# mosesyhc/LCGP

Hardware: AMD Instinct MI355X
Metric: NLL+grad evals/sec (higher is better)
Workload: dtype f64; 1 GPU; configs[2]: n=4096 d=6 p=64 q=8 submethod=full, one NLL+gradient evaluation per step; n=4096, d=6, p=64, q=8, parallelism=latent components k -> rank k mod 1, q_local_rank0=8

## Files before the change

lcgp_amd/csrc/lcgp_hip.hip:

```cpp
#include <hip/hip_runtime.h>
#include <stdint.h>
#include <stdio.h>
#include <string.h>
#include <math.h>
#include <type_traits>
#include <vector>

#include "../../include/lcgp_hip.h"
#include "fill_sched.h"
#include "sobol_subset.h"

#define LCGP_VERSION 610

namespace {

constexpr int TS = 64;
constexpr int KT = 16;
constexpr int DMAX = 32;
constexpr int DWIDE = 126;

typedef double d4 __attribute__((ext_vector_type(4)));
typedef float f4 __attribute__((ext_vector_type(4)));

thread_local char g_err[256] = "";
// ... 376 lines not shown
        out[(size_t)gi * ldo + gj] = (T)v;
    }
}

constexpr double MARG_SERIES_BELOW = 0.5;
constexpr int MARG_SERIES_TERMS = 20;

template <int KERN>
__device__ __forceinline__ void marg_series(double b, double& F, double& G) {
    double t = 1.0, sf = 0.0, sg = 0.0;
    for (int m = 0; m < MARG_SERIES_TERMS; ++m) {
        const double f = KERN == 0 ? 1.0 - m : (m - 1.0) * (m - 3.0) / 3.0;
        sf += t * f / (m + 1.0);
        sg += t * f / (m + 2.0);
        t *= -b / (m + 1.0);
    }
    F = b * sf;
    G = b * b * sg;
}

template <int KERN>
__device__ __forceinline__ double marg_F(double b) {
    if constexpr (KERN == 1) {
        return 1.2533141373155003 * erf(b * 0.70710678118654752);
    } else {
        if (b < MARG_SERIES_BELOW) { double F, G; marg_series<KERN>(b, F, G); return F; }
        const double e = exp(-b), em = -expm1(-b);
        if constexpr (KERN == 0) return 2.0 * em - b * e;
        else return (8.0 / 3.0) * em - b * (5.0 + b) / 3.0 * e;
    }
}

template <int KERN>
__device__ __forceinline__ double marg_G(double b) {
    if constexpr (KERN == 1) {
        return -expm1(-0.5 * b * b);
    } else {
        if (b < MARG_SERIES_BELOW) { double F, G; marg_series<KERN>(b, F, G); return G; }
        const double e = exp(-b), em = -expm1(-b);
        if constexpr (KERN == 0) return 3.0 * em - b * (3.0 + b) * e;
        else return 5.0 * em - b * (5.0 + b * (2.0 + b / 3.0)) * e;
    }
}

template <int KERN>
__device__ __forceinline__ double marg_Fc(double b) {
    if constexpr (KERN == 0) return (2.0 + b) * exp(-b);
    else if constexpr (KERN == 1) return 1.2533141373155003 * erfc(b * 0.70710678118654752);
    else return (8.0 + b * (5.0 + b)) / 3.0 * exp(-b);
}

template <int KERN>
__device__ __forceinline__ double marg_I1(double xv, double lo, double hi, double ell) {
    const double w = hi - lo;
    const double a1 = xv - lo, a2 = hi - xv;
    const double b1 = fabs(a1) / ell, b2 = fabs(a2) / ell;
    double r;
    if (a1 >= 0.0 && a2 >= 0.0) {
        r = marg_F<KERN>(b1) + marg_F<KERN>(b2);
    } else {
        const double bn = fmin(b1, b2), bf = fmax(b1, b2);
        r = bn > 1.0 ? marg_Fc<KERN>(bn) - marg_Fc<KERN>(bf) : marg_F<KERN>(bf) - marg_F<KERN>(bn);
    }
    return ell / w * r;
}

template <typename T, int KERN>
__global__ __launch_bounds__(256) void marg_table_kernel(const T* __restrict__ x, int n, int npad, int d,
                                                         const double* __restrict__ theta, int tw,
                                                         const double* __restrict__ box ,
                                                         double* __restrict__ tab, double* __restrict__ i2) {
    const int j = blockIdx.x * 256 + threadIdx.x, l = blockIdx.y, k = blockIdx.z;
    const double ell = theta[(size_t)k * tw + l];
    const double lo = box[l], hi = box[d + l], w = hi - lo;
    if (j == 0) {
        const double a = w / ell;
        i2[(size_t)k * d + l] = 2.0 * (marg_F<KERN>(a) / a - marg_G<KERN>(a) / (a * a));
    }
    if (j >= npad) return;
    double v = 1.0;
    if (j < n) {
        v = marg_I1<KERN>((double)x[(size_t)j * d + l], lo, hi, ell);
    }
    tab[((size_t)k * d + l) * npad + j] = v;
}

__device__ __forceinline__ double fast_rcp(double a) {
    double x = __builtin_amdgcn_rcp(a);
    x = fma(fma(-a, x, 1.0), x, x);
    x = fma(fma(-a, x, 1.0), x, x);
    return x;
}

template <int C>
__device__ __forceinline__ double row_bcast(double x) {
    double o;
    asm("s_nop 1\n\tv_mov_b64_dpp %0, %1 row_newbcast:%2 row_mask:0xf bank_mask:0xf" : "=v"(o) : "v"(x), "n"(C));
    return o;
}

template <int C>
__device__ __forceinline__ void fmac_row_bcast(double& acc, double u, double v) {
    asm("v_fmac_f64_dpp %0, %1, %2 row_newbcast:%3 row_mask:0xf bank_mask:0xf" : "+v"(acc) : "v"(u), "v"(v), "n"(C));
}

template <int S, int C>
struct PivotCols {
    static __device__ __forceinline__ void run(double (&rD)[16], double (&rL)[16], double vD, double vL) {
        if constexpr (C < 16) {
            fmac_row_bcast<C>(rD[C], rD[S], vD);
            fmac_row_bcast<C>(rL[C], rD[S], vL);
            PivotCols<S, C + 1>::run(rD, rL, vD, vL);
        }
    }
};

template <int S>
struct PivotSteps {
    static __device__ __forceinline__ void run(double (&rD)[16], double (&rL)[16], double& dmine, int i) {
        if constexpr (S < 16) {
            const double dp = row_bcast<S>(rD[S]);
            dmine = i == S ? rD[S] : dmine;
            const double rdp = fast_rcp(dp);
            const double vD = -rD[S] * rdp, vL = -rL[S] * rdp;
            PivotCols<S, S + 1>::run(rD, rL, vD, vL);
            PivotSteps<S + 1>::run(rD, rL, dmine, i);
        }
    }
};

template <int S>
struct ScaleCols {
    static __device__ __forceinline__ void run(double (&rD)[16], double (&rL)[16], double rsl) {
        if constexpr (S < 16) {
            const double f = row_bcast<S>(rsl);
            rD[S] *= f;
            rL[S] *= f;
            ScaleCols<S + 1>::run(rD, rL, rsl);
        }
    }
};

__device__ __forceinline__ double fast_rsqrt(double a) {
    double y = __builtin_amdgcn_rsq(a);
    double e = fma(-(a * y), y, 1.0);
    y = fma(0.5 * y, e, y);
    e = fma(-(a * y), y, 1.0);
    y = fma(0.5 * y, e, y);
    return y;
}

constexpr int LEAF_LDT = TS + 1;
constexpr int LEAF_SCR = TS * 17;
constexpr int LEAF_LDS_BYTES = (2 * TS * LEAF_LDT + LEAF_SCR + 2 * TS) * 8 + 16;

__device__ __forceinline__ void leaf_inverse_diag(double (*lt)[LEAF_LDT], double (*w)[LEAF_LDT], const double* dinv, int a,
                                                  int lane) {
    if (lane < 16) {
        const int b0 = a * 16, cl = lane;
        double wc[16];
#pragma unroll
        for (int i = 0; i < 16; ++i) {
            double sacc = i == cl ? -1.0 : 0.0;
#pragma unroll
            for (int m = 0; m < i; ++m) sacc = fma(lt[b0 + m][b0 + i], wc[m], sacc);
            wc[i] = -sacc * dinv[b0 + i];
        }
#pragma unroll
        for (int i = 0; i < 16; ++i) w[b0 + i][b0 + cl] = wc[i];
    }
}

__device__ __forceinline__ d4 leaf_inverse_t(double (*lt)[LEAF_LDT], double (*w)[LEAF_LDT], int a, int b, int lane) {
    const int li = lane & 15, lq = lane >> 4;
    d4 tacc = {0.0, 0.0, 0.0, 0.0};
    for (int mb = b; mb < a; ++mb) {
#pragma unroll
        for (int st = 0; st < 4; ++st)
            tacc = __builtin_amdgcn_mfma_f64_16x16x4f64(lt[mb * 16 + 4 * st + lq][a * 16 + li], w[mb * 16 + 4 * st + lq][b * 16 + li],
                                                        tacc, 0, 0, 0);
    }
    return tacc;
}

__device__ __forceinline__ void leaf_inverse_w(double (*w)[LEAF_LDT], const d4& tacc, int a, int b, int lane) {
    const int li = lane & 15, lq = lane >> 4;
    d4 wacc = {0.0, 0.0, 0.0, 0.0};
#pragma unroll
    for (int st = 0; st < 4; ++st)
        wacc = __builtin_amdgcn_mfma_f64_16x16x4f64(w[a * 16 + li][a * 16 + 4 * st + lq], tacc[st], wacc, 0, 0, 0);
#pragma unroll
    for (int e = 0; e < 4; ++e) w[a * 16 + lq + 4 * e][b * 16 + li] = -wacc[e];
}

template <typename T>
__device__ __forceinline__ void leaf_store_l_panel(T* __restrict__ Mb, int npad, double (*lt)[LEAF_LDT], int pb, int lane) {
    const int col = pb * 16 + (lane & 15);
#pragma unroll
    for (int m = 0; m < 16; ++m) {
        const int i = (lane >> 4) + 4 * m;
        Mb[(size_t)i * npad + col] = (T)lt[col][i];
    }
}

template <typename T>
__device__ __forceinline__ void leaf_store_w_rows(T* __restrict__ Wb, int npad, double (*w)[LEAF_LDT], int a, int lane) {
#pragma unroll
    for (int m = 0; m < 16; ++m) {
        const int i = a * 16 + m;
        Wb[(size_t)i * npad + lane] = (T)(lane <= i ? w[i][lane] : 0.0);
    }
}

template <typename T, bool FROM_LDS>
__device__ __forceinline__ void leaf_factor_invert(T* __restrict__ Mb, T* __restrict__ Wb, int npad, double (*lt)[LEAF_LDT],
                                                   double (*w)[LEAF_LDT], double* scratch, double* dinv, double* pivs,
                                                   int* bad, int jb) {
    const int tid = body_tid(), lane = tid & 63, wv = __builtin_amdgcn_readfirstlane(tid >> 6);
    const int li = lane & 15, lq = lane >> 4;
    d4 acc[4];
#pragma unroll
    for (int rb = 0; rb < 4; ++rb)
#pragma unroll
        for (int e = 0; e < 4; ++e)
            acc[rb][e] = rb < wv ? 0.0 : FROM_LDS ? w[rb * 16 + lq + 4 * e][wv * 16 + li]
                                                  : (double)Mb[(size_t)(rb * 16 + lq + 4 * e) * npad + wv * 16 + li];
    double (*S)[17] = (double (*)[17])scratch;
    int first_bad = 0;
#pragma unroll 1
    for (int kb = 0; kb < 4; ++kb) {
        if (wv == kb) {
#pragma unroll
            for (int rb = 0; rb < 4; ++rb)
#pragma unroll
                for (int e = 0; e < 4; ++e)
                    if (rb >= kb) S[rb * 16 + lq + 4 * e][li] = acc[rb][e];
            const int nlow = 3 - kb;
            const int base = kb * 16;
            double rD[16], rL[16];
            const int lrow = lq < nlow ? base + 16 * (1 + lq) + li : base + li;
#pragma unroll
            for (int c = 0; c < 16; ++c) {
                rD[c] = S[base + li][c];
                const double below = S[lrow][c];
                rL[c] = lq < nlow ? below : 0.0;
            }
            double dmine = 1.0;
            PivotSteps<0>::run(rD, rL, dmine, li);
            const double rsl = fast_rsqrt(dmine);
            ScaleCols<0>::run(rD, rL, rsl);
            if (lq == 0) { dinv[base + li] = rsl; pivs[base + li] = dmine; }
            const unsigned long long bm = __ballot(!(dmine > 0.0)) & 0xffffull;
            if (bm) first_bad = jb * TS + base + __ffsll((long long)bm);
            const int row = lq < nlow ? base + 16 * (1 + lq) + li : lq == nlow ? base + li : 16 * (lq - nlow - 1) + li;
#pragma unroll
            for (int m = 0; m < 16; ++m)
                lt[base + m][row] = lq < nlow ? rL[m] : (lq == nlow && li >= m) ? rD[m] : 0.0;
            if (lane == 0) bad[kb] = first_bad;
        } else if (wv == kb - 1) {
            const int a = kb - 1;
            leaf_inverse_diag(lt, w, dinv, a, lane);
            for (int b = 0; b < a; ++b) {
                const d4 tacc = leaf_inverse_t(lt, w, a, b, lane);
                leaf_inverse_w(w, tacc, a, b, lane);
            }
        } else if (kb == 0) {
            if ((jb & 1) == 0)
                for (int i = wv - 1; i < TS; i += 3) Wb[(size_t)i * npad + TS + lane] = (T)0;
        } else if (wv == ((kb + 1) & 3)) {
            leaf_store_l_panel<T>(Mb, npad, lt, kb - 1, lane);
        } else if (kb >= 2 && wv == ((kb + 2) & 3)) {
            leaf_store_w_rows<T>(Wb, npad, w, kb - 2, lane);
        }
        __syncthreads();
        if (wv > kb) {
#pragma unroll
            for (int st = 0; st < 4; ++st) {
                const double bv = lt[kb * 16 + 4 * st + lq][wv * 16 + li];
#pragma unroll
                for (int rb = 1; rb < 4; ++rb)
                    if (rb >= wv)
                        acc[rb] = __builtin_amdgcn_mfma_f64_16x16x4f64(-lt[kb * 16 + 4 * st + lq][rb * 16 + li], bv, acc[rb],
                                                                       0, 0, 0);
            }
        }
    }
    d4 tacc = {0.0, 0.0, 0.0, 0.0};
    if (wv == 3) leaf_inverse_diag(lt, w, dinv, 3, lane);
    else tacc = leaf_inverse_t(lt, w, 3, wv, lane);
    __syncthreads();
    if (wv < 3) leaf_inverse_w(w, tacc, 3, wv, lane);
    else leaf_store_l_panel<T>(Mb, npad, lt, 3, lane);
    __syncthreads();
    if (wv == 1) leaf_store_w_rows<T>(Wb, npad, w, 2, lane);
    else if (wv == 2) leaf_store_w_rows<T>(Wb, npad, w, 3, lane);
}

template <typename T, bool FROM_LDS = false>
__device__ __forceinline__ void leaf_body(unsigned char* lds, int k, T* __restrict__ M, T* __restrict__ W, size_t mat,
                                          int npad, int jb, double* __restrict__ logdet, int* __restrict__ info) {
    double (*lt)[LEAF_LDT] = (double (*)[LEAF_LDT])lds;
    double (*w)[LEAF_LDT] = (double (*)[LEAF_LDT])((double*)lds + TS * LEAF_LDT);
    double* scratch = (double*)lds + 2 * TS * LEAF_LDT;
    double* dinv = scratch + LEAF_SCR;
    double* pivs = dinv + TS;
    int* bad = (int*)(pivs + TS);
    const int tid = body_tid();
    T* Mb = M + (size_t)k * mat + (size_t)jb * TS * npad + (size_t)jb * TS;
    T* Wb = W + (size_t)k * mat + (size_t)jb * TS * npad + (size_t)jb * TS;
    double ld_prev = 0.0;
    int info_prev = 0;
    if (tid == 0) { ld_prev = logdet[k]; info_prev = info[k]; }
    leaf_factor_invert<T, FROM_LDS>(Mb, Wb, npad, lt, w, scratch, dinv, pivs, bad, jb);
    if (tid < TS) {
        double lg = 0.5 * log(pivs[tid]);
        for (int off = 32; off > 0; off >>= 1) lg += __shfl_xor(lg, off);
        if (tid == 0) {
            logdet[k] = ld_prev + lg;
            const int fb = bad[0] ? bad[0] : bad[1] ? bad[1] : bad[2] ? bad[2] : bad[3];
            if (fb && info_prev == 0) info[k] = fb;
        }
    }
}

template <typename T>
__global__ __launch_bounds__(256, 2) void leaf_kernel(T* __restrict__ M, T* __restrict__ W, size_t mat, int npad, int jb,
                                                   double* __restrict__ logdet, int* __restrict__ info) {
    __shared__ __align__(16) unsigned char lds[LEAF_LDS_BYTES];
    leaf_body<T>(lds, blockIdx.x, M, W, mat, npad, jb, logdet, info);
}

enum GemmOp { OP_SYRK = 1, OP_TRTRI_T = 2, OP_TRTRI_W = 3, OP_LAUUM = 4, OP_PRED_U = 5, OP_PRED_COV = 6, OP_PRED_V = 7, OP_VR = 8,
              OP_VG_P = 9, OP_VG_G = 10, OP_HESS_G = 11, OP_COND_CROSS = 12, OP_COND_U = 13 };
enum Lay { MK = 0, KM = 1 };

struct GemmArgs {
    const void* A; const void* B; void* C;
    size_t sA, sB, sC;
    int ldA, ldB, ldC;
    int nb;
    int p0, p1, p2, p3;
    int q;
    int t0;
    int skipq;
    const void* bvec = nullptr;
    double* part = nullptr;
    unsigned long long* clk = nullptr;
    const double* theta = nullptr;
    const void* xa = nullptr;
    const void* xb = nullptr;
    const double* wref = nullptr;
    const double* gvc = nullptr;
    int ldg = 0, d = 0, kern = 0, tw = 0, nrep = 1, ldp = 0;
};

template <typename T>
__device__ __forceinline__ constexpr int lds_swz(int k) { return (k & 12) * (int)(8 / sizeof(T)); }
static_assert(KT == 16, "lds_swz assumes 16 k rows per stage");
template <typename T>
__device__ __forceinline__ int swz_col(int g16, int l15, int kk) {
    return (g16 ^ (lds_swz<T>(4 * kk) & ~15)) + (l15 ^ (lds_swz<T>(4 * kk) & 15));
}

template <typename T, int L, int TM, int NT>
__device__ __forceinline__ void load_stage(const T* __restrict__ P, int ld, int ks, T (&reg)[TM * KT / NT], int tid) {
    constexpr int EPT = TM * KT / NT;
    if (L == MK) {
        constexpr int TPR = KT / EPT;
        const int m = tid / TPR, kk = (tid % TPR) * EPT;
        const T* src = P + (size_t)m * ld + ks + kk;
#pragma unroll
        for (int e = 0; e < EPT; ++e) reg[e] = src[e];
    } else {
        constexpr int TPK = TM / EPT;
        constexpr int PE = 16 / (int)sizeof(T), NP = EPT / PE;
        const int kq = tid / TPK, j = tid % TPK;
        const T* src = P + (size_t)(ks + kq) * ld + j * PE;
#pragma unroll
        for (int pc = 0; pc < NP; ++pc)
#pragma unroll
            for (int e = 0; e < PE; ++e) reg[pc * PE + e] = src[pc * (TM / NP) + e];
    }
}

template <typename T, int L, int TM, int NT>
__device__ __forceinline__ void store_stage(T* __restrict__ S, const T (&reg)[TM * KT / NT], int tid) {
    constexpr int EPT = TM * KT / NT;
    constexpr int LD = TM + 16;
    if (L == MK) {
        constexpr int TPR = KT / EPT;
        const int m = tid / TPR, kk = (tid % TPR) * EPT;
#pragma unroll
        for (int e = 0; e < EPT; ++e) S[(kk + e) * LD + (m ^ lds_swz<T>(kk + e))] = reg[e];
    } else {
        constexpr int TPK = TM / EPT;
        constexpr int PE = 16 / (int)sizeof(T), NP = EPT / PE;
        const int kq = tid / TPK, j = tid % TPK;
#pragma unroll
        for (int pc = 0; pc < NP; ++pc)
#pragma unroll
            for (int e = 0; e < PE; ++e) S[kq * LD + ((j * PE + pc * (TM / NP)) ^ lds_swz<T>(kq)) + e] = reg[pc * PE + e];
    }
}

template <typename T> struct Piece;
template <> struct Piece<double> { typedef double v __attribute__((ext_vector_type(2))); };
template <> struct Piece<float> { typedef float v __attribute__((ext_vector_type(4))); };

template <int IMM, typename P>
__device__ __forceinline__ void gload_piece(P& dst, unsigned voff, const void* sbase) {
    asm volatile("global_load_dwordx4 %0, %1, %2 offset:%3" : "=v"(dst) : "v"(voff), "s"(sbase), "n"(IMM) : "memory");
}

template <int N, typename P>
__device__ __forceinline__ void vm_wait_set(P (&a)[1], P (&b)[1]) {
    asm volatile("s_waitcnt vmcnt(%2)" : "+v"(a[0]), "+v"(b[0]) : "n"(N) : "memory");
}
template <int N, typename P>
__device__ __forceinline__ void vm_wait_set(P (&a)[4], P (&b)[4]) {
    asm volatile("s_waitcnt vmcnt(%8)" : "+v"(a[0]), "+v"(a[1]), "+v"(a[2]), "+v"(a[3]), "+v"(b[0]), "+v"(b[1]), "+v"(b[2]), "+v"(b[3])
                 : "n"(N) : "memory");
}
template <int N, typename P>
__device__ __forceinline__ void vm_wait_set(P (&a)[2], P (&b)[2]) {
    asm volatile("s_waitcnt vmcnt(%4)" : "+v"(a[0]), "+v"(a[1]), "+v"(b[0]), "+v"(b[1]) : "n"(N) : "memory");
}

template <typename T, int L, int TM, int NT>
__device__ __forceinline__ unsigned stage_lane_offset(int ld, int tid) {
    constexpr int EPT = TM * KT / NT;
    constexpr int PE = 16 / (int)sizeof(T);
    if (L == MK) {
        constexpr int TPR = KT / EPT;
        const int m = tid / TPR, kk = (tid % TPR) * EPT;
        return (unsigned)((m * ld + kk) * (int)sizeof(T));
    } else {
        constexpr int TPK = TM / EPT;
        const int kq = tid / TPK, j = tid % TPK;
        return (unsigned)((kq * ld + j * PE) * (int)sizeof(T));
    }
}

template <typename T, int L, int TM, int NT>
__device__ __forceinline__ void load_stage_u(const T* __restrict__ P , int ld, int ks, T (&reg)[TM * KT / NT],
                                             unsigned voff) {
    constexpr int EPT = TM * KT / NT;
    const T* src = (const T*)((const char*)(L == MK ? P + ks : P + (size_t)ks * ld) + voff);
    if (L == MK) {
#pragma unroll
        for (int e = 0; e < EPT; ++e) reg[e] = src[e];
    } else {
        constexpr int PE = 16 / (int)sizeof(T), NP = EPT / PE;
#pragma unroll
        for (int pc = 0; pc < NP; ++pc)
#pragma unroll
            for (int e = 0; e < PE; ++e) reg[pc * PE + e] = src[pc * (TM / NP) + e];
    }
}

template <typename T, int L, int TM, int NT, int PC = 0>
__device__ __forceinline__ void load_stage_p(const T* __restrict__ P , int ld, int ks,
                                             typename Piece<T>::v (&reg)[TM * KT / NT * (int)sizeof(T) / 16], unsigned voff) {
    constexpr int EPT = TM * KT / NT;
    constexpr int PE = 16 / (int)sizeof(T), NP = EPT / PE;
    const T* base = L == MK ? P + ks : P + (size_t)ks * ld;
    constexpr int STEP = (L == MK ? PE : TM / NP) * (int)sizeof(T);
    if constexpr (PC < NP) {
        gload_piece<PC * STEP>(reg[PC], voff, base);
        load_stage_p<T, L, TM, NT, PC + 1>(P, ld, ks, reg, voff);
    }
}

template <typename T, int L, int TM, int NT>
__device__ __forceinline__ void store_stage_p(T* __restrict__ S, const typename Piece<T>::v (&reg)[TM * KT / NT * (int)sizeof(T) / 16],
                                              int tid) {
// ... 719 lines not shown

template <typename T>
struct Tile64 {
    typedef typename Mfma<T>::acc_t acc_t;
    static constexpr int LD = TS + 16, NT = 256, EPT = TS * KT / NT, SPT = TS / KT;
    static __device__ __forceinline__ void load(acc_t (&acc)[2][2], const T* Ct, int ld, int lane, int wm0, int wn0) {
#pragma unroll
        for (int i = 0; i < 2; ++i)
#pragma unroll
            for (int j = 0; j < 2; ++j)
#pragma unroll
                for (int e = 0; e < 4; ++e)
                    acc[i][j][e] = Ct[(size_t)(wm0 + i * 16 + Mfma<T>::row(lane, e)) * ld + wn0 + j * 16 + (lane & 15)];
    }
    static __device__ __forceinline__ void zero(acc_t (&acc)[2][2]) {
#pragma unroll
        for (int i = 0; i < 2; ++i)
#pragma unroll
            for (int j = 0; j < 2; ++j)
#pragma unroll
                for (int e = 0; e < 4; ++e) acc[i][j][e] = 0;
    }
    static __device__ __forceinline__ void store(const acc_t (&acc)[2][2], T* Ct, int ld, int lane, int wm0, int wn0) {
#pragma unroll
        for (int i = 0; i < 2; ++i)
#pragma unroll
            for (int j = 0; j < 2; ++j)
#pragma unroll
                for (int e = 0; e < 4; ++e)
                    Ct[(size_t)(wm0 + i * 16 + Mfma<T>::row(lane, e)) * ld + wn0 + j * 16 + (lane & 15)] = (T)acc[i][j][e];
    }
    static __device__ __forceinline__ void fetch(T (&p)[SPT][EPT], const T* P, int ld, int tid) {
#pragma unroll
        for (int s = 0; s < SPT; ++s) load_stage<T, MK, TS, NT>(P, ld, s * KT, p[s], tid);
    }
    template <bool NEG>
    static __device__ __forceinline__ void mma_regs(acc_t (&acc)[2][2], const T (&pa)[SPT][EPT], const T (&pb)[SPT][EPT],
                                                    T* lds, int tid, int lane, int wm0, int wn0) {
        T* As = lds;
        T* Bs = As + 2 * KT * LD;
#pragma unroll
        for (int s = 0; s < SPT; ++s) {
            store_stage<T, MK, TS, NT>(As + (s & 1) * KT * LD, pa[s], tid);
            store_stage<T, MK, TS, NT>(Bs + (s & 1) * KT * LD, pb[s], tid);
            __syncthreads();
            const T* as = As + (s & 1) * KT * LD;
            const T* bs = Bs + (s & 1) * KT * LD;
#pragma unroll
            for (int kk = 0; kk < KT / 4; ++kk) {
                const int krow = (kk * 4 + (lane >> 4)) * LD;
                T af[2], bf[2];
#pragma unroll
                for (int i = 0; i < 2; ++i) {
                    const T v = as[krow + wm0 + swz_col<T>(i * 16, lane & 15, kk)];
                    af[i] = NEG ? -v : v;
                }
#pragma unroll
                for (int j = 0; j < 2; ++j) bf[j] = bs[krow + wn0 + swz_col<T>(j * 16, lane & 15, kk)];
#pragma unroll
                for (int i = 0; i < 2; ++i)
#pragma unroll
                    for (int j = 0; j < 2; ++j) acc[i][j] = Mfma<T>::run(af[i], bf[j], acc[i][j]);
            }
        }
    }
    template <bool NEG>
    static __device__ __forceinline__ void mma(acc_t (&acc)[2][2], const T* A0, int ldA, const T* B0, int ldB, T* lds,
                                               int tid, int lane, int wm0, int wn0) {
        T pa[SPT][EPT], pb[SPT][EPT];
        fetch(pa, A0, ldA, tid);
        fetch(pb, B0, ldB, tid);
        mma_regs<NEG>(acc, pa, pb, lds, tid, lane, wm0, wn0);
    }
    static __device__ __forceinline__ void to_operand(const acc_t (&acc)[2][2], T* F, int lane, int wm0, int wn0) {
#pragma unroll
        for (int i = 0; i < 2; ++i)
#pragma unroll
            for (int j = 0; j < 2; ++j)
#pragma unroll
                for (int e = 0; e < 4; ++e)
                    F[(wn0 + j * 16 + (lane & 15)) * LD + ((wm0 + i * 16 + Mfma<T>::row(lane, e)) ^ (lane & 15))] = acc[i][j][e];
    }
    template <bool NEG>
    static __device__ __forceinline__ void mma_a_lds(acc_t (&acc)[2][2], const T* F, const T (&pb)[SPT][EPT], T* Bs, int tid,
                                                     int lane, int wm0, int wn0) {
#pragma unroll
        for (int s = 0; s < SPT; ++s) {
            store_stage<T, MK, TS, NT>(Bs + (s & 1) * KT * LD, pb[s], tid);
            __syncthreads();
            const T* as = F + s * KT * LD;
            const T* bs = Bs + (s & 1) * KT * LD;
#pragma unroll
            for (int kk = 0; kk < KT / 4; ++kk) {
                const int krow = (kk * 4 + (lane >> 4)) * LD;
                T af[2], bf[2];
#pragma unroll
                for (int i = 0; i < 2; ++i) {
                    const T v = as[krow + wm0 + i * 16 + ((lane & 15) ^ (4 * kk + (lane >> 4)))];
                    af[i] = NEG ? -v : v;
                }
#pragma unroll
                for (int j = 0; j < 2; ++j) bf[j] = bs[krow + wn0 + swz_col<T>(j * 16, lane & 15, kk)];
#pragma unroll
                for (int i = 0; i < 2; ++i)
#pragma unroll
                    for (int j = 0; j < 2; ++j) acc[i][j] = Mfma<T>::run(af[i], bf[j], acc[i][j]);
            }
        }
    }
    template <bool NEG>
    static __device__ __forceinline__ void mma_ab_lds(acc_t (&acc)[2][2], const T* F, int lane, int wm0, int wn0) {
#pragma unroll
        for (int kk = 0; kk < TS / 4; ++kk) {
            const int krow = (kk * 4 + (lane >> 4)) * LD;
            T af[2], bf[2];
#pragma unroll
            for (int i = 0; i < 2; ++i) {
                const T v = F[krow + wm0 + i * 16 + ((lane & 15) ^ ((4 * kk + (lane >> 4)) & 15))];
                af[i] = NEG ? -v : v;
            }
#pragma unroll
            for (int j = 0; j < 2; ++j) bf[j] = F[krow + wn0 + j * 16 + ((lane & 15) ^ ((4 * kk + (lane >> 4)) & 15))];
#pragma unroll
            for (int i = 0; i < 2; ++i)
#pragma unroll
                for (int j = 0; j < 2; ++j) acc[i][j] = Mfma<T>::run(af[i], bf[j], acc[i][j]);
        }
    }
};

template <typename T>
__device__ __forceinline__ void chain_step_body(const StepArgs& a, int b, unsigned char* lds) {
    typedef Tile64<T> TL;
    const int tid = body_tid(), lane = tid & 63, wave = __builtin_amdgcn_readfirstlane(tid >> 6);
    const int wm0 = (wave >> 1) * 32, wn0 = (wave & 1) * 32;
    const int ld = a.npad;
    const int nspecial = a.has_special * a.q;
    int t = -1, k = 0;
    if (b < nspecial) { t = 0; k = b; }
    else if (b < nspecial + a.fs.nblk) { fill_dispatch<T>(a.fs, b - nspecial, lds); return; }
    else {
        b -= nspecial + a.fs.nblk;
        if (b < (a.n_trmm - a.has_special) * a.q) { k = b % a.q; t = b / a.q + a.has_special; }
        else b -= (a.n_trmm - a.has_special) * a.q;
    }
    if (t >= 0) {
        if (t == 0 && a.has_special) __builtin_amdgcn_s_setprio(3);
        const int c = a.c, r = a.trmm_r0 + t;
        T* Mk = (T*)a.M + (size_t)k * a.mat;
        const T* Wk = (const T*)a.W + (size_t)k * a.mat;
        T* Ct = Mk + (size_t)r * TS * ld + (size_t)c * TS;
        T* F = (T*)lds;
        T* Bst = F + TS * TL::LD;
        typename TL::acc_t acc[2][2];
        T pw[TL::SPT][TL::EPT];
        TL::fetch(pw, Wk + (size_t)c * TS * ld + (size_t)c * TS, ld, tid);
        TL::load(acc, Ct, ld, lane, wm0, wn0);
        if (c > a.J) {
            TL::template mma<true>(acc, Mk + (size_t)r * TS * ld + (size_t)(c - 1) * TS, ld,
                                   Mk + (size_t)c * TS * ld + (size_t)(c - 1) * TS, ld, (T*)lds, tid, lane, wm0, wn0);
            __syncthreads();
        }
        TL::to_operand(acc, F, lane, wm0, wn0);
        TL::zero(acc);
        TL::template mma_a_lds<false>(acc, F, pw, Bst, tid, lane, wm0, wn0);
        TL::store(acc, Ct, ld, lane, wm0, wn0);
        if (r < a.diag_end) {
            T* Dt = Mk + (size_t)r * TS * ld + (size_t)r * TS;
            typename TL::acc_t dacc[2][2];
            TL::load(dacc, Dt, ld, lane, wm0, wn0);
            __syncthreads();
            TL::to_operand(acc, F, lane, wm0, wn0);
            __syncthreads();
            TL::template mma_ab_lds<true>(dacc, F, lane, wm0, wn0);
            if (a.has_special && t == 0) {
                __syncthreads();
                double (*blk)[LEAF_LDT] = (double (*)[LEAF_LDT])((double*)lds + TS * LEAF_LDT);
#pragma unroll
                for (int i = 0; i < 2; ++i)
#pragma unroll
                    for (int j = 0; j < 2; ++j)
#pragma unroll
                        for (int e = 0; e < 4; ++e)
                            blk[wm0 + i * 16 + Mfma<T>::row(lane, e)][wn0 + j * 16 + (lane & 15)] = (double)dacc[i][j][e];
                __syncthreads();
                leaf_body<T, true>(lds, k, (T*)a.M, (T*)a.W, a.mat, a.npad, c + 1, a.logdet, a.info);
            } else {
                TL::store(dacc, Dt, ld, lane, wm0, wn0);
            }
        }
        return;
    }
    {
        k = b % a.q;
        t = b / a.q;
        const int cc = a.c + 1;
        const int r = a.upd_r0 + t;
        T* Mk = (T*)a.M + (size_t)k * a.mat;
        T* Ct = Mk + (size_t)r * TS * ld + (size_t)cc * TS;
        typename TL::acc_t acc[2][2];
        TL::load(acc, Ct, ld, lane, wm0, wn0);
        T pa[2][TL::SPT][TL::EPT], pb[2][TL::SPT][TL::EPT];
        const T* Ar = Mk + (size_t)r * TS * ld;
        const T* Br = Mk + (size_t)cc * TS * ld;
        TL::fetch(pa[0], Ar + (size_t)a.J * TS, ld, tid);
        TL::fetch(pb[0], Br + (size_t)a.J * TS, ld, tid);
        for (int j = a.J; j < a.c; j += 2) {
            if (j + 1 < a.c) {
                TL::fetch(pa[1], Ar + (size_t)(j + 1) * TS, ld, tid);
                TL::fetch(pb[1], Br + (size_t)(j + 1) * TS, ld, tid);
            }
            TL::template mma_regs<true>(acc, pa[0], pb[0], (T*)lds, tid, lane, wm0, wn0);
            if (j + 1 < a.c) {
                if (j + 2 < a.c) {
                    TL::fetch(pa[0], Ar + (size_t)(j + 2) * TS, ld, tid);
                    TL::fetch(pb[0], Br + (size_t)(j + 2) * TS, ld, tid);
                }
                TL::template mma_regs<true>(acc, pa[1], pb[1], (T*)lds, tid, lane, wm0, wn0);
            }
        }
        TL::store(acc, Ct, ld, lane, wm0, wn0);
    }
}

template <typename T>
__global__ __launch_bounds__(256, 2) void chain_step_kernel(StepArgs a) {
    __shared__ __align__(16) unsigned char lds[LEAF_LDS_BYTES];
    chain_step_body<T>(a, blockIdx.x, lds);
}

template <typename T, int TM>
__global__ __launch_bounds__(256, 2) void wide_leaf_kernel(GemmArgs g, T* __restrict__ M, T* __restrict__ W, size_t mat,
                                                           int npad, int jb, double* __restrict__ logdet,
                                                           int* __restrict__ info) {
    constexpr int WIDE_LDS = 4 * KT * (TM + 16) * (int)sizeof(T);
    __shared__ __align__(16) unsigned char lds[WIDE_LDS > LEAF_LDS_BYTES ? WIDE_LDS : LEAF_LDS_BYTES];
    const int q = g.q;
    if ((int)blockIdx.x < q) {
        leaf_body<T>(lds, blockIdx.x, M, W, mat, npad, jb, logdet, info);
        return;
    }
    gemm_body<T, OP_SYRK, TM, 4>(g, blockIdx.x - q, lds);
}

template <typename T>
__global__ __launch_bounds__(256) void symv_tile_kernel(const T* __restrict__ V, size_t mat, int npad,
                                                        const T* __restrict__ b, double* __restrict__ part, int ntile) {
    __shared__ double vt[TS][TS + 1];
    __shared__ double red[4][TS];
    __shared__ double br[TS], bc[TS];
    const int k = blockIdx.y;
    int r, c;
    tri_decode(blockIdx.x, r, c);
    const T* Vt = V + (size_t)k * mat + (size_t)r * TS * npad + (size_t)c * TS;
    const int tid = threadIdx.x, j = tid & 63, g = tid >> 6;
    if (tid < TS) {
        br[tid] = (double)b[(size_t)k * npad + r * TS + tid];
        bc[tid] = (double)b[(size_t)k * npad + c * TS + tid];
    }
    double v[16];
#pragma unroll
    for (int m = 0; m < 16; ++m) v[m] = (double)Vt[(size_t)(g * 16 + m) * npad + j];
    __syncthreads();
    double* dst = part + ((size_t)k * ntile + blockIdx.x) * 2 * TS;
    double s2 = 0.0;
#pragma unroll
    for (int m = 0; m < 16; ++m) {
        s2 = fma(v[m], br[g * 16 + m], s2);
        vt[g * 16 + m][j] = v[m];
    }
    red[g][j] = s2;
    __syncthreads();
    if (tid < TS) dst[TS + tid] = r == c ? 0.0 : (red[0][tid] + red[1][tid]) + (red[2][tid] + red[3][tid]);
    double s1 = 0.0;
#pragma unroll
    for (int m = 0; m < 16; ++m) s1 = fma(vt[j][g * 16 + m], bc[g * 16 + m], s1);
    __syncthreads();
    red[g][j] = s1;
    __syncthreads();
    if (tid < TS) dst[tid] = (red[0][tid] + red[1][tid]) + (red[2][tid] + red[3][tid]);
}

template <typename T, int TZ>
__global__ __launch_bounds__(256) void symv_reduce_kernel(const double* __restrict__ part, int ntile, int npad, int nb,
                                                          T* __restrict__ z) {
    constexpr int NG = 256 / TZ;
    __shared__ double sh[NG][TZ];
    const int k = blockIdx.y, R = blockIdx.x, i = threadIdx.x % TZ, g = threadIdx.x / TZ;
    const double* pk = part + (size_t)k * ntile * 2 * TZ;
    double s = 0.0;
    for (int c = g; c <= R; c += NG) s += pk[((size_t)(R * (R + 1) / 2 + c)) * 2 * TZ + i];
    for (int r = R + 1 + g; r < nb; r += NG) s += pk[((size_t)(r * (r + 1) / 2 + R)) * 2 * TZ + TZ + i];
    sh[g][i] = s;
    __syncthreads();
    if (g == 0) {
        double v;
        if constexpr (NG == 4) v = (sh[0][i] + sh[1][i]) + (sh[2][i] + sh[3][i]);
        else v = sh[0][i] + sh[1][i];
        z[(size_t)k * npad + R * TZ + i] = (T)v;
    }
}

__device__ __forceinline__ double block_sum(double v, double* sh , int tid) {
    for (int off = 32; off > 0; off >>= 1) v += __shfl_xor(v, off);
    __syncthreads();
    if ((tid & 63) == 0) sh[tid >> 6] = v;
    __syncthreads();
    return (sh[0] + sh[1]) + (sh[2] + sh[3]);
}

template <typename T>
__device__ __forceinline__ void gsig_body(int a, int k, int n, int npad, int d, int p, const T* __restrict__ Y,
                                          const T* __restrict__ b, const T* __restrict__ z, double* __restrict__ out) {
    __shared__ double sh[4];
    const int tid = threadIdx.x;
    const T* bk = b + (size_t)k * npad;
    const T* zk = z + (size_t)k * npad;
    double s = 0.0;
    for (int i = tid; i < n; i += 256) s += (double)Y[(size_t)a * n + i] * ((double)bk[i] - (double)zk[i]);
    s = block_sum(s, sh, tid);
    if (tid == 0) out[(size_t)k * (d + 5 + p) + 5 + d + a] = s;
}

template <typename T, int DD, int KERN>
__global__ __launch_bounds__(256) void grad_kernel(const T* __restrict__ V, size_t mat, int n, int npad, int d, int p,
                                                   const T* __restrict__ x, const T* __restrict__ sr,
                                                   const T* __restrict__ z, const double* __restrict__ theta,
                                                   double* __restrict__ part, int ntile, const T* __restrict__ Y,
                                                   const T* __restrict__ bvec, double* __restrict__ out,
                                                   double* __restrict__ cpart) {
    constexpr bool CZ = sizeof(T) == 4;
    if ((int)blockIdx.x >= ntile) {
        gsig_body<T>(blockIdx.x - ntile, blockIdx.y, n, npad, d, p, Y, bvec, z, out);
        return;
    }
    __shared__ double xr[TS][DD + 1];
    __shared__ double xc[TS][DD + 1];
    __shared__ double zr[TS], zc[TS], srr[TS], src[TS];
    __shared__ double red[4][DD + 2];
// ... 6606 lines not shown
```

Measured before the change: 94.44 evals/s.

## Restructure leaf Cholesky/inverse to cut LDS round-trips and barriers

Reworks the 64x64 leaf factor-and-invert. The diagonal inverse now takes the factored rows from registers, with cross-lane row broadcasts, instead of re-reading LDS and a dinv array. Panel updates preload their operands before the MFMAs, and the first pivot block reads straight from the source, skipping the scratch copy. Part of the final inverse work is overlapped with the last iteration, the logdet reduction is folded into an idle wave, and the last W block is written directly to global memory, removing one barrier. Also moves the diagonal tile load earlier in the chained TRMM kernel and gives blk its own LDS region so a sync can be dropped. The cost is more complex LDS aliasing and extra register pressure.

```diff
diff --git a/lcgp_amd/csrc/lcgp_hip.hip b/lcgp_amd/csrc/lcgp_hip.hip
--- a/lcgp_amd/csrc/lcgp_hip.hip
+++ b/lcgp_amd/csrc/lcgp_hip.hip
@@ -552,29 +552,47 @@
 
 constexpr int LEAF_LDT = TS + 1;
 constexpr int LEAF_SCR = TS * 17;
-constexpr int LEAF_LDS_BYTES = (2 * TS * LEAF_LDT + LEAF_SCR + 2 * TS) * 8 + 16;
-
-__device__ __forceinline__ void leaf_inverse_diag(double (*lt)[LEAF_LDT], double (*w)[LEAF_LDT], const double* dinv, int a,
-                                                  int lane) {
+constexpr int LEAF_LDS_BYTES = (2 * TS * LEAF_LDT + LEAF_SCR + TS) * 8 + 16;
+constexpr int CHAIN_BLK_OFF = TS * (TS + 16);
+
+template <int I, int M>
+struct InvDot {
+    static __device__ __forceinline__ void run(double& sacc, const double (&ld)[16], const double (&wc)[16]) {
+        if constexpr (M < I) {
+            fmac_row_bcast<I>(sacc, ld[M], wc[M]);
+            InvDot<I, M + 1>::run(sacc, ld, wc);
+        }
+    }
+};
+
+template <int I>
+struct InvRows {
+    static __device__ __forceinline__ void run(const double (&ld)[16], double rsl, double (&wc)[16], int cl) {
+        if constexpr (I < 16) {
+            double sacc = I == cl ? -1.0 : 0.0;
+            InvDot<I, 0>::run(sacc, ld, wc);
+            wc[I] = -sacc * row_bcast<I>(rsl);
+            InvRows<I + 1>::run(ld, rsl, wc, cl);
+        }
+    }
+};
+
+__device__ __forceinline__ void leaf_inverse_diag(const d4 (&lrow)[4], double rsl, double (*w)[LEAF_LDT], int a, int lane) {
+    const int b0 = a * 16, cl = lane & 15;
+    double ld[16], wc[16];
+#pragma unroll
+    for (int m = 0; m < 16; ++m) ld[m] = lrow[m >> 2][m & 3];
+    InvRows<0>::run(ld, rsl, wc, cl);
     if (lane < 16) {
-        const int b0 = a * 16, cl = lane;
-        double wc[16];
-#pragma unroll
-        for (int i = 0; i < 16; ++i) {
-            double sacc = i == cl ? -1.0 : 0.0;
-#pragma unroll
-            for (int m = 0; m < i; ++m) sacc = fma(lt[b0 + m][b0 + i], wc[m], sacc);
-            wc[i] = -sacc * dinv[b0 + i];
-        }
 #pragma unroll
         for (int i = 0; i < 16; ++i) w[b0 + i][b0 + cl] = wc[i];
     }
 }
 
-__device__ __forceinline__ d4 leaf_inverse_t(double (*lt)[LEAF_LDT], double (*w)[LEAF_LDT], int a, int b, int lane) {
+__device__ __forceinline__ d4 leaf_inverse_t(double (*lt)[LEAF_LDT], double (*w)[LEAF_LDT], int a, int b, int lane, int mb0,
+                                             int mb1, d4 tacc) {
     const int li = lane & 15, lq = lane >> 4;
-    d4 tacc = {0.0, 0.0, 0.0, 0.0};
-    for (int mb = b; mb < a; ++mb) {
+    for (int mb = mb0; mb < mb1; ++mb) {
 #pragma unroll
         for (int st = 0; st < 4; ++st)
             tacc = __builtin_amdgcn_mfma_f64_16x16x4f64(lt[mb * 16 + 4 * st + lq][a * 16 + li], w[mb * 16 + 4 * st + lq][b * 16 + li],
@@ -583,6 +601,10 @@
     return tacc;
 }
 
+__device__ __forceinline__ d4 leaf_inverse_t(double (*lt)[LEAF_LDT], double (*w)[LEAF_LDT], int a, int b, int lane) {
+    return leaf_inverse_t(lt, w, a, b, lane, b, a, d4{0.0, 0.0, 0.0, 0.0});
+}
+
 __device__ __forceinline__ void leaf_inverse_w(double (*w)[LEAF_LDT], const d4& tacc, int a, int b, int lane) {
     const int li = lane & 15, lq = lane >> 4;
     d4 wacc = {0.0, 0.0, 0.0, 0.0};
@@ -612,44 +634,96 @@
     }
 }
 
+template <typename T>
+__device__ __forceinline__ void leaf_inverse_w_store(T* __restrict__ Wb, int npad, double (*w)[LEAF_LDT], const d4& tacc, int b,
+                                                     int lane) {
+    const int li = lane & 15, lq = lane >> 4;
+    d4 wacc = {0.0, 0.0, 0.0, 0.0};
+#pragma unroll
+    for (int st = 0; st < 4; ++st)
+        wacc = __builtin_amdgcn_mfma_f64_16x16x4f64(w[48 + li][48 + 4 * st + lq], tacc[st], wacc, 0, 0, 0);
+#pragma unroll
+    for (int e = 0; e < 4; ++e) Wb[(size_t)(48 + lq + 4 * e) * npad + b * 16 + li] = (T)(-wacc[e]);
+}
+
+template <typename T>
+__device__ __forceinline__ void leaf_store_w33(T* __restrict__ Wb, int npad, double (*w)[LEAF_LDT], int lane) {
+    const int li = lane & 15, lq = lane >> 4;
+#pragma unroll
+    for (int e = 0; e < 4; ++e) {
+        const int i = lq + 4 * e;
+        Wb[(size_t)(48 + i) * npad + 48 + li] = (T)(li <= i ? w[48 + i][48 + li] : 0.0);
+    }
+}
+
+template <int WV>
+__device__ __forceinline__ void leaf_apply_panel(d4 (&acc)[4], const double* lk) {
+    double bv[4], av[4][4];
+#pragma unroll
+    for (int st = 0; st < 4; ++st) {
+        bv[st] = lk[4 * st * LEAF_LDT + WV * 16];
+#pragma unroll
+        for (int rb = WV; rb < 4; ++rb) av[st][rb] = -lk[4 * st * LEAF_LDT + rb * 16];
+    }
+#pragma unroll
+    for (int st = 0; st < 4; ++st)
+#pragma unroll
+        for (int rb = WV; rb < 4; ++rb) acc[rb] = __builtin_amdgcn_mfma_f64_16x16x4f64(av[st][rb], bv[st], acc[rb], 0, 0, 0);
+}
+
 template <typename T, bool FROM_LDS>
 __device__ __forceinline__ void leaf_factor_invert(T* __restrict__ Mb, T* __restrict__ Wb, int npad, double (*lt)[LEAF_LDT],
-                                                   double (*w)[LEAF_LDT], double* scratch, double* dinv, double* pivs,
-                                                   int* bad, int jb) {
+                                                   double (*w)[LEAF_LDT], const double (*blk)[LEAF_LDT], double* scratch,
+                                                   double* pivs, int* bad, int jb, int k,
+                                                   double* __restrict__ logdet, int* __restrict__ info) {
     const int tid = body_tid(), lane = tid & 63, wv = __builtin_amdgcn_readfirstlane(tid >> 6);
     const int li = lane & 15, lq = lane >> 4;
+    double ld_prev = 0.0;
+    int info_prev = 0;
+    if (tid == 64) { ld_prev = logdet[k]; info_prev = info[k]; }
     d4 acc[4];
-#pragma unroll
-    for (int rb = 0; rb < 4; ++rb)
-#pragma unroll
-        for (int e = 0; e < 4; ++e)
-            acc[rb][e] = rb < wv ? 0.0 : FROM_LDS ? w[rb * 16 + lq + 4 * e][wv * 16 + li]
-                                                  : (double)Mb[(size_t)(rb * 16 + lq + 4 * e) * npad + wv * 16 + li];
+    if (wv != 0) {
+#pragma unroll
+        for (int rb = 0; rb < 4; ++rb)
+#pragma unroll
+            for (int e = 0; e < 4; ++e)
+                acc[rb][e] = rb < wv ? 0.0 : FROM_LDS ? blk[rb * 16 + lq + 4 * e][wv * 16 + li]
+                                                      : (double)Mb[(size_t)(rb * 16 + lq + 4 * e) * npad + wv * 16 + li];
+    }
     double (*S)[17] = (double (*)[17])scratch;
     int first_bad = 0;
+    double rsl_mine = 0.0;
+    d4 tacc = {0.0, 0.0, 0.0, 0.0};
 #pragma unroll 1
     for (int kb = 0; kb < 4; ++kb) {
         if (wv == kb) {
-#pragma unroll
-            for (int rb = 0; rb < 4; ++rb)
-#pragma unroll
-                for (int e = 0; e < 4; ++e)
-                    if (rb >= kb) S[rb * 16 + lq + 4 * e][li] = acc[rb][e];
             const int nlow = 3 - kb;
             const int base = kb * 16;
             double rD[16], rL[16];
             const int lrow = lq < nlow ? base + 16 * (1 + lq) + li : base + li;
-#pragma unroll
-            for (int c = 0; c < 16; ++c) {
-                rD[c] = S[base + li][c];
-                const double below = S[lrow][c];
-                rL[c] = lq < nlow ? below : 0.0;
+            if (kb == 0) {
+#pragma unroll
+                for (int c = 0; c < 16; ++c) {
+                    rD[c] = FROM_LDS ? blk[li][c] : (double)Mb[(size_t)li * npad + c];
+                    rL[c] = FROM_LDS ? blk[lrow][c] : (double)Mb[(size_t)lrow * npad + c];
+                }
+            } else {
+#pragma unroll
+                for (int rb = 0; rb < 4; ++rb)
+#pragma unroll
+                    for (int e = 0; e < 4; ++e)
+                        if (rb >= kb) S[rb * 16 + lq + 4 * e][li] = acc[rb][e];
+#pragma unroll
+                for (int c = 0; c < 16; ++c) {
+                    rD[c] = S[base + li][c];
+                    rL[c] = S[lrow][c];
+                }
             }
             double dmine = 1.0;
             PivotSteps<0>::run(rD, rL, dmine, li);
             const double rsl = fast_rsqrt(dmine);
             ScaleCols<0>::run(rD, rL, rsl);
-            if (lq == 0) { dinv[base + li] = rsl; pivs[base + li] = dmine; }
+            if (lq == 0) pivs[base + li] = dmine;
             const unsigned long long bm = __ballot(!(dmine > 0.0)) & 0xffffull;
             if (bm) first_bad = jb * TS + base + __ffsll((long long)bm);
             const int row = lq < nlow ? base + 16 * (1 + lq) + li : lq == nlow ? base + li : 16 * (lq - nlow - 1) + li;
@@ -657,9 +731,12 @@
             for (int m = 0; m < 16; ++m)
                 lt[base + m][row] = lq < nlow ? rL[m] : (lq == nlow && li >= m) ? rD[m] : 0.0;
             if (lane == 0) bad[kb] = first_bad;
+#pragma unroll
+            for (int m = 0; m < 16; ++m) acc[m >> 2][m & 3] = rD[m];
+            rsl_mine = rsl;
         } else if (wv == kb - 1) {
             const int a = kb - 1;
-            leaf_inverse_diag(lt, w, dinv, a, lane);
+            leaf_inverse_diag(acc, rsl_mine, w, a, lane);
             for (int b = 0; b < a; ++b) {
                 const d4 tacc = leaf_inverse_t(lt, w, a, b, lane);
                 leaf_inverse_w(w, tacc, a, b, lane);
@@ -672,55 +749,50 @@
         } else if (kb >= 2 && wv == ((kb + 2) & 3)) {
             leaf_store_w_rows<T>(Wb, npad, w, kb - 2, lane);
         }
+        if (kb == 3 && wv < 2) tacc = leaf_inverse_t(lt, w, 3, wv, lane, wv, 2, tacc);
         __syncthreads();
         if (wv > kb) {
-#pragma unroll
-            for (int st = 0; st < 4; ++st) {
-                const double bv = lt[kb * 16 + 4 * st + lq][wv * 16 + li];
-#pragma unroll
-                for (int rb = 1; rb < 4; ++rb)
-                    if (rb >= wv)
-                        acc[rb] = __builtin_amdgcn_mfma_f64_16x16x4f64(-lt[kb * 16 + 4 * st + lq][rb * 16 + li], bv, acc[rb],
-                                                                       0, 0, 0);
-            }
-        }
-    }
-    d4 tacc = {0.0, 0.0, 0.0, 0.0};
-    if (wv == 3) leaf_inverse_diag(lt, w, dinv, 3, lane);
-    else tacc = leaf_inverse_t(lt, w, 3, wv, lane);
+            const double* lk = &lt[kb * 16 + lq][li];
+            if (wv == 1) leaf_apply_panel<1>(acc, lk);
+            else if (wv == 2) leaf_apply_panel<2>(acc, lk);
+            else leaf_apply_panel<3>(acc, lk);
+        }
+    }
+    if (wv == 3) leaf_inverse_diag(acc, rsl_mine, w, 3, lane);
+    else tacc = leaf_inverse_t(lt, w, 3, wv, lane, 2, 3, tacc);
+    if (wv == 2) {
+        leaf_store_w_rows<T>(Wb, npad, w, 2, lane);
+    } else if (wv == 1) {
+        double lg = 0.5 * log(pivs[lane]);
+        for (int off = 32; off > 0; off >>= 1) lg += __shfl_xor(lg, off);
+        if (lane == 0) {
+            logdet[k] = ld_prev + lg;
+            const int fb = bad[0] ? bad[0] : bad[1] ? bad[1] : bad[2] ? bad[2] : bad[3];
+            if (fb && info_prev == 0) info[k] = fb;
+        }
+    }
     __syncthreads();
-    if (wv < 3) leaf_inverse_w(w, tacc, 3, wv, lane);
-    else leaf_store_l_panel<T>(Mb, npad, lt, 3, lane);
-    __syncthreads();
-    if (wv == 1) leaf_store_w_rows<T>(Wb, npad, w, 2, lane);
-    else if (wv == 2) leaf_store_w_rows<T>(Wb, npad, w, 3, lane);
+    if (wv < 3) {
+        leaf_inverse_w_store<T>(Wb, npad, w, tacc, wv, lane);
+    } else {
+        leaf_store_w33<T>(Wb, npad, w, lane);
+        leaf_store_l_panel<T>(Mb, npad, lt, 3, lane);
+    }
 }
 
 template <typename T, bool FROM_LDS = false>
 __device__ __forceinline__ void leaf_body(unsigned char* lds, int k, T* __restrict__ M, T* __restrict__ W, size_t mat,
-                                          int npad, int jb, double* __restrict__ logdet, int* __restrict__ info) {
+                                          int npad, int jb, double* __restrict__ logdet, int* __restrict__ info,
+                                          const double* blk = nullptr) {
     double (*lt)[LEAF_LDT] = (double (*)[LEAF_LDT])lds;
     double (*w)[LEAF_LDT] = (double (*)[LEAF_LDT])((double*)lds + TS * LEAF_LDT);
     double* scratch = (double*)lds + 2 * TS * LEAF_LDT;
-    double* dinv = scratch + LEAF_SCR;
-    double* pivs = dinv + TS;
+    double* pivs = scratch + LEAF_SCR;
     int* bad = (int*)(pivs + TS);
-    const int tid = body_tid();
     T* Mb = M + (size_t)k * mat + (size_t)jb * TS * npad + (size_t)jb * TS;
     T* Wb = W + (size_t)k * mat + (size_t)jb * TS * npad + (size_t)jb * TS;
-    double ld_prev = 0.0;
-    int info_prev = 0;
-    if (tid == 0) { ld_prev = logdet[k]; info_prev = info[k]; }
-    leaf_factor_invert<T, FROM_LDS>(Mb, Wb, npad, lt, w, scratch, dinv, pivs, bad, jb);
-    if (tid < TS) {
-        double lg = 0.5 * log(pivs[tid]);
-        for (int off = 32; off > 0; off >>= 1) lg += __shfl_xor(lg, off);
-        if (tid == 0) {
-            logdet[k] = ld_prev + lg;
-            const int fb = bad[0] ? bad[0] : bad[1] ? bad[1] : bad[2] ? bad[2] : bad[3];
-            if (fb && info_prev == 0) info[k] = fb;
-        }
-    }
+    leaf_factor_invert<T, FROM_LDS>(Mb, Wb, npad, lt, w, (const double (*)[LEAF_LDT])blk, scratch, pivs, bad, jb, k,
+                                    logdet, info);
 }
 
 template <typename T>
@@ -1746,8 +1818,9 @@
         T* Ct = Mk + (size_t)r * TS * ld + (size_t)c * TS;
         T* F = (T*)lds;
         T* Bst = F + TS * TL::LD;
-        typename TL::acc_t acc[2][2];
+        typename TL::acc_t acc[2][2], dacc[2][2];
         T pw[TL::SPT][TL::EPT];
+        T* Dt = Mk + (size_t)r * TS * ld + (size_t)r * TS;
         TL::fetch(pw, Wk + (size_t)c * TS * ld + (size_t)c * TS, ld, tid);
         TL::load(acc, Ct, ld, lane, wm0, wn0);
         if (c > a.J) {
@@ -1755,21 +1828,21 @@
                                    Mk + (size_t)c * TS * ld + (size_t)(c - 1) * TS, ld, (T*)lds, tid, lane, wm0, wn0);
             __syncthreads();
         }
+        if (r < a.diag_end) TL::load(dacc, Dt, ld, lane, wm0, wn0);
         TL::to_operand(acc, F, lane, wm0, wn0);
         TL::zero(acc);
         TL::template mma_a_lds<false>(acc, F, pw, Bst, tid, lane, wm0, wn0);
         TL::store(acc, Ct, ld, lane, wm0, wn0);
         if (r < a.diag_end) {
-            T* Dt = Mk + (size_t)r * TS * ld + (size_t)r * TS;
-            typename TL::acc_t dacc[2][2];
-            TL::load(dacc, Dt, ld, lane, wm0, wn0);
             __syncthreads();
             TL::to_operand(acc, F, lane, wm0, wn0);
             __syncthreads();
             TL::template mma_ab_lds<true>(dacc, F, lane, wm0, wn0);
             if (a.has_special && t == 0) {
-                __syncthreads();
-                double (*blk)[LEAF_LDT] = (double (*)[LEAF_LDT])((double*)lds + TS * LEAF_LDT);
+                static_assert(TS * TL::LD * sizeof(T) <= CHAIN_BLK_OFF * sizeof(double), "blk overlaps F");
+                static_assert(CHAIN_BLK_OFF >= TS * LEAF_LDT, "blk overlaps lt");
+                static_assert(CHAIN_BLK_OFF + TS * LEAF_LDT <= 2 * TS * LEAF_LDT + LEAF_SCR, "blk overlaps pivs");
+                double (*blk)[LEAF_LDT] = (double (*)[LEAF_LDT])((double*)lds + CHAIN_BLK_OFF);
 #pragma unroll
                 for (int i = 0; i < 2; ++i)
 #pragma unroll
@@ -1778,7 +1851,7 @@
                         for (int e = 0; e < 4; ++e)
                             blk[wm0 + i * 16 + Mfma<T>::row(lane, e)][wn0 + j * 16 + (lane & 15)] = (double)dacc[i][j][e];
                 __syncthreads();
-                leaf_body<T, true>(lds, k, (T*)a.M, (T*)a.W, a.mat, a.npad, c + 1, a.logdet, a.info);
+                leaf_body<T, true>(lds, k, (T*)a.M, (T*)a.W, a.mat, a.npad, c + 1, a.logdet, a.info, &blk[0][0]);
             } else {
                 TL::store(dacc, Dt, ld, lane, wm0, wn0);
             }
```

After: 95.42 evals/s (median of 3 runs). No clear change (+1.0%).
